# chenhanpolyu/fuxi-planner

Measured on AMD Instinct MI355X. Metric: start->goal plans/sec on 1024x1024 grid, higher is better.
Workload: dtype f64

## Files before the change

### fuxi-planner_amd/_lib.py

```python
import ctypes as C
import os

_HERE = os.path.dirname(os.path.abspath(__file__))
LIB_PATH = os.environ.get("FXJPS_LIB") or os.path.join(_HERE, "libfxjps.so")

OK = 0
E_ARG, E_NODEV, E_HIP, E_NOGRID, E_NOMEM, E_COMM = -1, -2, -3, -4, -5, -6
Q_NOPATH, Q_PATH_TOO_LONG, Q_BAD_START, Q_CAPACITY = 0, -1, -2, -3
BACKEND_HIP = 1

VERSION = 870
PATH_VALID, PATH_EMPTY, PATH_BLOCKED, PATH_OUTSIDE, PATH_MALFORMED = 1, 0, 2, 3, -1
SYMBOLS = ("fxjps_version", "fxjps_timing_size", "fxjps_last_timing_sized", "fxjps_rank_preflight", "fxjps_reserve_grid",
           "fxjps_device_count", "fxjps_create", "fxjps_rank_unique_id", "fxjps_create_rank", "fxjps_set_grid_rank", "fxjps_destroy", "fxjps_last_error",
           "fxjps_set_grid", "fxjps_set_grid_device", "fxjps_prepare_grid", "fxjps_prepare_occupancy_msg", "fxjps_get_grid", "fxjps_get_grid_context", "fxjps_publish_map", "fxjps_set_grid_image", "fxjps_snapshot_image", "fxjps_update_cells", "fxjps_update_cells_deferred", "fxjps_set_queries", "fxjps_replan_frame", "fxjps_plan_batch",
           "fxjps_plan_batch_csr", "fxjps_last_cells", "fxjps_last_timing", "fxjps_last_timing_device", "fxjps_comm_info", "fxjps_set_memory_share", "fxjps_selftest_sqrt", "fxjps_selftest_wavemin", "fxjps_selftest_openlist", "fxjps_debug_read_nbmask", "fxjps_debug_read_maps", "fxjps_debug_counters", "fxjps_debug_qstat",
           "fxjps_waypoint_st", "fxjps_waypoint_ccst", "fxjps_waypoint_ccst_batch", "fxjps_waypoint_st_batch",
           "fxjps_set_grid_slot", "fxjps_get_grid_slot", "fxjps_plan_batch_slots_csr", "fxjps_debug_read_slot_maps", "fxjps_debug_read_sets", "fxjps_debug_live_bytes",
           "fxjps_prepare_slots", "fxjps_slot_job_size", "fxjps_waypoint_slots_batch", "fxjps_publish_slots", "fxjps_slot_publish_size",
           "fxjps_tick_outputs_slots", "fxjps_refresh_slots", "fxjps_debug_read_slot_context", "fxjps_replan_slots",
           "fxjps_set_prior_map", "fxjps_get_prior_map", "fxjps_prepare_slots_world", "fxjps_refresh_slots_world", "fxjps_world_job_size",
           "fxjps_prepare_slots_cropped", "fxjps_refresh_slots_cropped", "fxjps_crop_size",
           "fxjps_refresh_grid", "fxjps_refresh_occupancy_msg", "fxjps_last_refresh_cells", "fxjps_replan_frame_raw",
           "fxjps_set_grid_slots", "fxjps_refresh_grid_slots", "fxjps_grid_job_size",
           "fxjps_set_slot_reuse", "fxjps_debug_slot_tiles", "fxjps_debug_slot_read_sets",
           "fxjps_check_path", "fxjps_check_paths_slots",
# ... 2 lines not shown
           "fxjps_absorb_prior_slide", "fxjps_slide_check", "fxjps_prior_keep_size", "fxjps_prior_slid_size")
MAX_GRID_SLOTS = 256
MAX_PRIOR_MAPS = 16
ABSORB_OVERWRITE, ABSORB_OCCUPIED, ABSORB_KNOWN = 0, 1, 2
ABSORB_MODES = {"overwrite": ABSORB_OVERWRITE, "occupied": ABSORB_OCCUPIED, "known": ABSORB_KNOWN}
KEEP_NONE, KEEP_ALWAYS, KEEP_OVER_LIMIT = 0, 1, 2
KEEP_USES = {"none": KEEP_NONE, "always": KEEP_ALWAYS, "over_limit": KEEP_OVER_LIMIT}
JOB_NOT_PLANNED = 1


class Timing(C.Structure):
    _fields_ = [("search_kernel_ms", C.c_double), ("total_ms", C.c_double), ("search_launches", C.c_int64),
                ("retried", C.c_int64), ("pops", C.c_int64), ("pushes", C.c_int64), ("far_refills", C.c_int64),
                ("slow_pops", C.c_int64), ("table_wipes", C.c_int64), ("reused", C.c_int64), ("table_direct", C.c_int64),
                ("waves", C.c_int64), ("waves_short", C.c_int64), ("head_launch_ms", C.c_double), ("batch_launch_ms", C.c_double),
                ("solo_timeouts", C.c_int64)]


class SlotJob(C.Structure):
    _fields_ = [("raw", C.c_void_p), ("slot", C.c_int32), ("layout", C.c_int32), ("W0", C.c_int32), ("H0", C.c_int32),
                ("ifa", C.c_int32), ("variant", C.c_int32), ("start_xy", C.c_int32 * 2), ("goal_xy", C.c_int32 * 2),
                ("W", C.c_int32), ("H", C.c_int32), ("map_d", C.c_int32 * 2), ("end_occu", C.c_int32), ("status", C.c_int32)]


class GridJob(C.Structure):
    _fields_ = [("occ", C.POINTER(C.c_uint8)), ("slot", C.c_int32), ("W", C.c_int32), ("H", C.c_int32), ("reserved", C.c_int32)]


class WorldJob(C.Structure):
    _fields_ = [("raw", C.c_void_p), ("slot", C.c_int32), ("layout", C.c_int32), ("W0", C.c_int32), ("H0", C.c_int32),
                ("ifa", C.c_int32), ("variant", C.c_int32), ("prior", C.c_int32), ("status", C.c_int32),
# ... 283 lines not shown
```

### fuxi-planner_amd/csrc/fxjps.hip

```cpp
#include <hip/hip_runtime.h>

#include <dlfcn.h>

#include <algorithm>
#include <atomic>
#include <chrono>
#include <cmath>
#include <cstdarg>
#include <cstddef>
#include <cstdio>
#include <cstdlib>
#include <cstring>
#include <mutex>
#include <string>
#include <thread>
#include <vector>

#include "../../include/fxjps.h"
#include "fxjps_kernels.hip.inc"
#include "fxjps_owned.h"
#include "fxjps_results.h"

namespace {

using fx::FarEnt;
using fx::GridDev;
using fx::SearchArgs;
using fx::TEnt;

thread_local std::string g_create_error;

bool dbg_on() {
    static int on = -1;
// ... 87 lines not shown
            **w = 0u;
            g_live_pinned += BYTES;
        } else {
            *w = nullptr;
        }
        return e;
    }
    static void destroy(uint32_t* w) {
        (void)hipHostFree(w);
        g_live_pinned -= BYTES;
    }
};
using Stream = fx::Owned<StreamRes>;
using Event = fx::Owned<EventRes>;
using MappedWord = fx::Owned<MappedWordRes>;

struct ScratchCfg {
    uint32_t nwaves = 0;
    uint32_t nbuckets = 0;
    uint32_t usable = 0;
    uint32_t direct_ly = 0;
    uint32_t far_cap = 0;
};

struct GridBufs {
    int W = 0, H = 0, PW = 0, PH = 0, NS = 0, LINES = 0, WORDS = 0, tsh = 0;
    DBuf<uint8_t> occ, nb8;
    DBuf<fx::BmWord> bm;
    DBuf<int> comp;
    DBuf<uint16_t> ci;
// ... 110 lines not shown
    std::vector<uint32_t> h_order;
    int64_t q0 = 0, nq = 0;
    int wall_khz = 100000;
    struct RunStats {
        double kernel_ms = 0;
        int64_t launches = 0, retried = 0;
        int64_t nrun = 0;
        uint32_t waves_used = 0;
        bool waves_short = false;
        bool had_solo = false;
        double head_ms = 0, batch_ms = 0;
    } run;
    HBuf<uint8_t> h_absorb_in;
    DBuf<uint8_t> d_absorb_in;
    HBuf<unsigned long long> h_absorb_out;

    DevCtx() = default;
    DevCtx(DevCtx&&) = default;
    DevCtx& operator=(DevCtx&&) = default;
    ~DevCtx() {
        if (dev < 0) return;
        (void)hipSetDevice(dev);
        if (stream_solo) (void)hipStreamSynchronize(stream_solo);
        if (stream) (void)hipStreamSynchronize(stream);
    }
};

}

struct fxjps {
    std::vector<DevCtx> devs;
    std::string err;
    std::mutex err_mu;
    bool have_grid = false;
    bool maps_stale = false;
    int mem_div = 1;
    fxjps_timing_t timing{};
// ... 60 lines not shown
        h->err = buf;
    } else {
        g_create_error = buf;
    }
    return code;
}

#define HIPCHK(h, call)                                                                          \
    do {                                                                                         \
        hipError_t e__ = (call);                                                                 \
        if (e__ != hipSuccess)                                                                   \
            return fail(h, e__ == hipErrorOutOfMemory ? FXJPS_E_NOMEM : FXJPS_E_HIP, "%s: %s (%s:%d)", \
                        #call, hipGetErrorString(e__), __FILE__, __LINE__);                      \
    } while (0)

uint32_t dirlut_entry(uint32_t pd, uint32_t nbm) {
    auto occ = [&](int dx, int dy) -> bool { return (nbm >> fx::nbit(dx, dy)) & 1u; };
    auto blocked = [&](int dx, int dy) -> bool {
        if (dx != 0 && dy != 0) return (occ(dx, 0) && occ(0, dy)) || occ(dx, dy);
        return occ(dx, dy);
    };
    uint32_t codes[8];
    int n = 0;
    auto add = [&](int dx, int dy) { codes[n++] = (uint32_t)((dx + 1) * 4 + (dy + 1)); };
    const int pdx = (int)(pd >> 2) - 1, pdy = (int)(pd & 3u) - 1;
    if (pd == fx::PD_NONE) {
        static const int all8[8][2] = {{-1, 0}, {0, -1}, {1, 0}, {0, 1}, {-1, -1}, {-1, 1}, {1, -1}, {1, 1}};
        for (auto& d : all8)
            if (!blocked(d[0], d[1])) add(d[0], d[1]);
    } else if (pdx < -1 || pdx > 1 || pdy < -1 || pdy > 1) {
    } else if (pdx != 0 && pdy != 0) {
        if (!blocked(0, pdy)) add(0, pdy);
        if (!blocked(pdx, 0)) add(pdx, 0);
        if ((!blocked(0, pdy) || !blocked(pdx, 0)) && !blocked(pdx, pdy)) add(pdx, pdy);
        if (blocked(-pdx, 0) && !blocked(0, pdy)) add(-pdx, pdy);
        if (blocked(0, -pdy) && !blocked(pdx, 0)) add(pdx, -pdy);
    } else if (pdx == 0) {
        if (!blocked(0, pdy)) add(0, pdy);
        if (blocked(1, 0)) add(1, pdy);
        if (blocked(-1, 0)) add(-1, pdy);
    } else {
        if (!blocked(pdx, 0)) {
            add(pdx, 0);
            if (blocked(0, 1)) add(pdx, 1);
            if (blocked(0, -1)) add(pdx, -1);
        }
    }
    uint32_t v = 0;
    for (int g = 0; g < 8; g++) v |= (g < n ? codes[g] : fx::DIR_NONE) << (4 * g);
    return v;
}

GridDev grid_of(const GridBufs& d) {
    GridDev G;
    G.bm = d.bm.p;
    G.ci = d.ci.p;
    G.nb8 = d.nb8.p;
    G.jd = d.jd.p;
    G.comp = d.comp.p;
    G.W = d.W;
    G.H = d.H;
    G.PW = d.PW;
    G.PH = d.PH;
    G.NS = d.NS;
    G.LINES = d.LINES;
    G.WORDS = d.WORDS;
    G.DLINES = d.PW + d.PH - 1;
    G.tsh = d.tsh;
    return G;
}

int derive_maps(fxjps* h, DevCtx& d, bool whole = true, GridBufs* slot = nullptr) {
    HIPCHK(h, hipSetDevice(d.dev));
    GridBufs& g = slot ? *slot : d;
    if (slot) whole = true;
    if (!whole && !d.dirty && !d.ccl_full) return FXJPS_OK;
    const bool box = !whole && d.dirty && (d.bx1 - d.bx0 + 1) * 2 <= g.PW && (d.by1 - d.by0 + 1) * 2 <= g.PH;
    const GridDev G = grid_of(g);
    const char* fused_env = getenv("FXJPS_FUSED_BUILD");
    if (whole && !(fused_env && atoi(fused_env) == 0) && (long long)g.W * g.H <= (1ll << 18)) {
        const long long ncell = (long long)g.W * g.H, npad = (long long)g.PW * g.PH;
        const unsigned nb_rows = (unsigned)(((long long)g.PW * g.WORDS + 3) / 4), nb_cols = (unsigned)(((long long)g.PH * g.WORDS + 3) / 4);
        const unsigned nb_cell = (unsigned)((ncell + 255) / 256), nb_ci = (unsigned)((npad + 255) / 256);
        const unsigned nb_diag = (unsigned)((4ll * G.DLINES * g.WORDS + 15) / 16), nb_flat = (unsigned)((ncell + 1023) / 1024);
        hipLaunchKernelGGL(fx::k_build_1, dim3(nb_rows + nb_cols + nb_cell), dim3(256), 0, d.stream, g.occ.p, G, g.nb8.p, g.bm.p, g.comp.p, nb_rows, nb_cols);
        hipLaunchKernelGGL(fx::k_build_2, dim3(nb_ci + nb_cell), dim3(256), 0, d.stream, g.occ.p, G, g.ci.p, g.comp.p, nb_ci);
        hipLaunchKernelGGL(fx::k_build_3, dim3(nb_diag + nb_flat), dim3(1024), 0, d.stream, g.occ.p, G, g.bm.p + (size_t)4 * g.LINES * g.WORDS, g.comp.p, nb_diag);
        hipLaunchKernelGGL(fx::k_derive_jd, dim3((unsigned)((npad * 8 + 255) / 256)), dim3(256), 0, d.stream, G, g.jd.p, fx::DiagRange{1, d.bx0, d.bx1, d.by0, d.by1});
        HIPCHK(h, hipGetLastError());
        if (!slot) {
// ... 107 lines not shown
    d.LINES = std::max(d.PW, d.PH);
    d.WORDS = (std::max(d.PW, d.PH) + 63) / 64;
    d.tsh = 0;
    while (((std::max(W, H) - 1) >> d.tsh) > 63) d.tsh++;
    HIPCHK(h, d.occ.ensure((size_t)W * H));
    HIPCHK(h, d.comp.ensure((size_t)W * H));
    HIPCHK(h, d.nb8.ensure((size_t)d.PW * d.NS));
    HIPCHK(h, d.ci.ensure((size_t)d.PW * d.NS));
    HIPCHK(h, d.jd.ensure((size_t)d.PW * d.NS * 8));
    HIPCHK(h, d.bm.ensure((size_t)4 * d.LINES * d.WORDS + (size_t)4 * (d.PW + d.PH - 1) * d.WORDS));
    return FXJPS_OK;
}

int alloc_grid(fxjps* h, DevCtx& d, int W, int H) {
    HIPCHK(h, hipSetDevice(d.dev));
    bool knob = false;
    for (const char* k : {"FXJPS_TABLE_LOG2", "FXJPS_TABLE_SHIFT", "FXJPS_FAR_CAP", "FXJPS_POOL_BUDGET_MB", "FXJPS_POOL_FRAC", "FXJPS_DIRECT",
                          "FXJPS_TABLE_SHRINK"})
        knob = knob || getenv(k) != nullptr;
    if (W != d.W || H != d.H || knob) {
        d.pool_clean[0] = d.pool_clean[1] = false;
        d.cfg[0] = ScratchCfg();
        d.cfg[1] = ScratchCfg();
        d.owner_ready = false;
        d.chg_ready = false;
    }
    return alloc_grid_bufs(h, d, W, H);
}

constexpr uint64_t wpb_down(uint64_t v) { return v / (uint64_t)fx::WPB * (uint64_t)fx::WPB; }
// ... 202 lines not shown
    A.max_pops = 64ull * (unsigned long long)req.cells + 4096ull;
    if (req.slots) {
        A.grids = d.d_slot_desc.p;
        A.grid_ids = d.d_grid_ids.p;
    }
    if (d.st.on) {
        A.host_cells = d.st.cells;
        A.host_cap = d.st.cap;
        A.host_cursor = d.d_cursor.p;
        A.host_base = d.st.base;
        A.host_len = d.st.len;
        A.host_cost = d.st.cost;
    }
}

int launch_search(fxjps* h, DevCtx& d, const BatchReq& req, int pool, const uint32_t* d_order, uint32_t nrun) {
    const ScratchCfg& c = d.cfg[pool];
    const bool track = req.track();
    SearchArgs A;
    fill_search_args(d, req, pool, A, d_order, nrun);
    uint32_t waves = std::min<uint32_t>(c.nwaves, (nrun + 0u));
    waves = std::max<uint32_t>((uint32_t)fx::WPB, (uint32_t)wpb_up(waves));
    waves = std::min<uint32_t>(waves, c.nwaves);
    uint32_t nsolo = (nrun <= 32768u && d.share * h->mem_div == 1) ? 16u : 0u, live_solo = 1, live_main = 0;
    if (const char* e = getenv("FXJPS_SOLO")) nsolo = (uint32_t)std::max(0, atoi(e));
    if (const char* e = getenv("FXJPS_SOLO_LIVE")) live_solo = (uint32_t)std::max(1, atoi(e));
    if (const char* e = getenv("FXJPS_SPREAD")) live_main = (uint32_t)std::max(0, atoi(e));
    if (live_solo != 1u && live_solo != 2u && live_solo != 4u) live_solo = 4u;
    if (live_main != 0u && live_main != 1u && live_main != 2u && live_main != 4u) live_main = 4u;
    if (pool != 0 || track || d_order == nullptr || d.solo_started == nullptr || d.solo_timeouts_run >= 3 || nrun < 4096u || nrun < 64u * nsolo ||
        waves <= 2u * nsolo + (uint32_t)fx::WPB)
        nsolo = 0;
    nsolo = std::min<uint32_t>(nsolo, 512u) & ~(live_solo - 1u);
    if (nsolo != 0u) waves = std::min<uint32_t>(waves, (uint32_t)wpb_down(c.nwaves - nsolo));

    if (pool != 0 || nsolo != 0u || (uint64_t)nrun > (uint64_t)d.n_cu * live_main || d.share * h->mem_div > 1) live_main = 0u;
    if (pool == 0) d.run.waves_used = waves;
    HIPCHK(h, hipMemsetAsync(d.d_next.p, 0, 4 * sizeof(unsigned int), d.stream));
    const dim3 block(fx::WAVE * fx::WPB);
    DBG("launch k_search pool=%d waves=%u nrun=%u buckets=%u far_cap=%u solo=%u x %u spread=%u", pool, waves, nrun, c.nbuckets, c.far_cap, nsolo,
        live_solo, live_main);
    HIPCHK(h, hipEventRecord(d.ev0, d.stream));
    {
        const SearchKernel k = search_kernel(req.hchoice, track, c.direct_ly > 0, req.slots);
        const SearchFn fn = k.fn;
        static const size_t pad = 36u << 10;
        if (nsolo != 0u || live_main != 0u) {
            if (!d.lds_attr_done[k.index]) {
                if (hipFuncSetAttribute(reinterpret_cast<const void*>(fn), hipFuncAttributeMaxDynamicSharedMemorySize, (int)pad) == hipSuccess) {
// ... 41 lines not shown
            hipLaunchKernelGGL(fn, dim3(waves / fx::WPB), block, 0, d.stream, A);
        }
        HIPCHK(h, hipGetLastError());
        if (nsolo != 0u) {
            HIPCHK(h, hipEventRecord(d.ev_bt1, d.stream));
            HIPCHK(h, hipStreamWaitEvent(d.stream, d.ev_solo1, 0));
        }
        if (pool == 0) d.run.had_solo = nsolo != 0u;
    }
    HIPCHK(h, hipEventRecord(d.ev1, d.stream));
    if (d.st.on) {
        hipLaunchKernelGGL(fx::k_counters_out, dim3(1), dim3(64), 0, d.stream, d.d_counters.p, d.st.counters);
        HIPCHK(h, hipGetLastError());
    }
    d.run.launches += nsolo != 0u ? 2 : 1;
    return FXJPS_OK;
}

constexpr size_t ARENA_BYTES = (size_t)1 << 30;
int begin_streaming(fxjps* h, DevCtx& d, const BatchReq& req) {
    const int64_t nq = d.nq;
    const unsigned long long limit = ARENA_BYTES / sizeof(uint32_t) / h->devs.size();
    unsigned long long want = (unsigned long long)nq * (unsigned long long)std::min(req.max_len, 512);
    want = std::max(want, (unsigned long long)d.arena_peak + (unsigned long long)d.arena_peak / 4);
    if (const char* e = getenv("FXJPS_ARENA_CELLS")) want = (unsigned long long)std::max(0ll, atoll(e));
    if (want > limit) return FXJPS_OK;
    HIPCHK(h, d.h_arena.ensure((size_t)std::max(want, 1ull)));
    HIPCHK(h, d.h_base.ensure((size_t)nq));
    HIPCHK(h, d.d_cursor.ensure(1));
    void *dp_cells = nullptr, *dp_base = nullptr, *dp_len = nullptr, *dp_cost = nullptr, *dp_cnt = nullptr;
// ... 82 lines not shown
    int rc = ensure_pool(h, d, req, 0, (uint32_t)std::min<int64_t>(full, (d.run.nrun + 3) & ~3ll));
    if (rc) return rc;
    DBG("pool ready");
    if (req.stream && d.cfg[0].direct_ly > 0)
        if ((rc = begin_streaming(h, d, req)) != FXJPS_OK) return rc;
    return launch_search(h, d, req, 0, d.d_order.p, (uint32_t)d.run.nrun);
}

int finish_search(fxjps* h, DevCtx& d, const BatchReq& req) {
    HIPCHK(h, hipSetDevice(d.dev));
    const int64_t nq = d.nq;
    if (nq == 0) return FXJPS_OK;
    DBG("waiting for the search kernel");
    HIPCHK(h, hipStreamSynchronize(d.stream));
    DBG("search kernel done");
    if (!d.st.on) {
        HIPCHK(h, hipMemcpyAsync(d.h_len.p, d.d_len.p, (size_t)nq * sizeof(int32_t), hipMemcpyDeviceToHost, d.stream));
        HIPCHK(h, hipStreamSynchronize(d.stream));
    }
    float ms = 0;
    if (d.run.launches > 0) {
        HIPCHK(h, hipEventElapsedTime(&ms, d.ev0, d.ev1));
        d.run.kernel_ms += ms;
        if (d.run.had_solo) {
            float a = 0, b = 0;
            HIPCHK(h, hipEventElapsedTime(&a, d.ev_hd0, d.ev_hd1));
            HIPCHK(h, hipEventElapsedTime(&b, d.ev_bt0, d.ev_bt1));
            d.run.head_ms = a;
            d.run.batch_ms = b;
        }
// ... 308 lines not shown
    T.search_kernel_ms = 0;
    T.search_launches = 0;
    T.retried = 0;
    T.pops = 0;
    T.pushes = 0;
    T.far_refills = 0;
    T.slow_pops = 0;
    T.table_wipes = 0;
    T.reused = 0;
    T.table_direct = 0;
    T.waves = 0;
    T.waves_short = 0;
    T.head_launch_ms = 0;
    T.batch_launch_ms = 0;
    T.solo_timeouts = 0;
    for (auto& d : h->devs) {
        T.head_launch_ms = std::max(T.head_launch_ms, d.run.head_ms);
        T.batch_launch_ms = std::max(T.batch_launch_ms, d.run.batch_ms);
        T.solo_timeouts += d.solo_timeouts;
        T.waves += d.run.waves_used;
        if (d.run.waves_short) T.waves_short = 1;
        T.search_kernel_ms = std::max(T.search_kernel_ms, d.run.kernel_ms);
        T.search_launches += d.run.launches;
        T.retried += d.run.retried;
        if (d.nq > 0) {
            T.pops += (int64_t)d.h_counters.p[0];
            T.pushes += (int64_t)d.h_counters.p[1];
            T.far_refills += (int64_t)d.h_counters.p[2];
            T.slow_pops += (int64_t)d.h_counters.p[3];
            T.table_wipes += (int64_t)d.h_counters.p[7];
            if (d.cfg[0].direct_ly > 0) T.table_direct = 1;
// ... 90 lines not shown
        if (rc) return rc;
    }
    for (auto& d : h->devs) {
        if (!wait) break;
        HIPCHK(h, hipSetDevice(d.dev));
        HIPCHK(h, hipStreamSynchronize(d.stream));
    }
    h->have_grid = true;
    h->maps_stale = false;
    return FXJPS_OK;
}

void drain_all(fxjps* h) {
    const std::string keep = h->err;
    for (auto& d : h->devs) {
        if (hipSetDevice(d.dev) == hipSuccess) {
            if (d.stream_solo) (void)hipStreamSynchronize(d.stream_solo);
            (void)hipStreamSynchronize(d.stream);
        }
        d.pool_clean[0] = d.pool_clean[1] = false;
        d.owner_ready = d.chg_ready = false;
    }
    (void)hipGetLastError();
    h->err = keep;
}

struct WpPaths {
    struct Part {
        DevCtx* d;
        int64_t q0, n, total, kept_at;
        const long long* h_off;
// ... 677 lines not shown
    HIPCHK(h, hipSetDevice(d.dev));
    const size_t n = (size_t)d.W * d.H * channels;
    HIPCHK(h, d.d_img.ensure(n));
    int rc = transpose_map(h, d, d.occ.p, d.W, d.H, 0, 1, fx::TM_OCC_TO_GRAY, channels, d.d_img.p);
    if (rc) return rc;
    HIPCHK(h, hipMemcpyAsync(out, d.d_img.p, n, hipMemcpyDeviceToHost, d.stream));
    HIPCHK(h, hipStreamSynchronize(d.stream));
    return FXJPS_OK;
}

namespace {
int update_cells_async(fxjps_t* h, const int32_t* xy, const uint8_t* val, int64_t n, bool derive) {
    if (!h->have_grid) return fail(h, FXJPS_E_NOGRID, "cell update before fxjps_set_grid");
    if (n < 0 || n > 0x7FFFFFF0ll || (n > 0 && (!xy || !val))) return fail(h, FXJPS_E_ARG, "bad update arrays");
    if (n == 0 && !(derive && h->maps_stale)) return FXJPS_OK;
    int bx0 = 0, bx1 = -1, by0 = 0, by1 = -1;
    bool have_box = false;
    {
        const DevCtx& d0 = h->devs[0];
        for (int64_t i = 0; i < n; i++) {
            const int x = xy[2 * i], y = xy[2 * i + 1];
            if (x < 0 || y < 0 || x >= d0.W || y >= d0.H) continue;
            bx0 = have_box ? std::min(bx0, x) : x;
            bx1 = have_box ? std::max(bx1, x) : x;
            by0 = have_box ? std::min(by0, y) : y;
            by1 = have_box ? std::max(by1, y) : y;
            have_box = true;
        }
    }
    static const bool partial = !(getenv("FXJPS_PARTIAL_DERIVE") && atoi(getenv("FXJPS_PARTIAL_DERIVE")) == 0);
// ... 2757 lines not shown
```

### fuxi-planner_amd/csrc/fxjps_kernels.hip.inc

```

namespace fx {

constexpr int WAVE = 64;
#define FX_RARE(c) __builtin_expect(!!(c), 0)
#define FX_USUAL(c) __builtin_expect(!!(c), 1)
#ifndef FXJPS_WPB
#define FXJPS_WPB 8
#endif
#ifndef FXJPS_OCC
#define FXJPS_OCC 4
#endif
constexpr int WPB = FXJPS_WPB;
constexpr int OCC = FXJPS_OCC;
constexpr uint32_t KEY_CLOSED = 0x80000000u;
constexpr uint32_t CELL_MASK = 0x03FFFFFFu;
constexpr uint32_t PD_NONE = 5;
constexpr uint32_t SLOT_NONE = 0xFFFFFFFFu;
constexpr uint32_t PAR_MASK = 0x07FFFFFFu;
constexpr uint32_t PAR_NONE = PAR_MASK;
constexpr uint32_t GEN_WRAP = 63u;
__host__ __device__ constexpr uint32_t ent_gen(uint32_t key, uint32_t par) { return ((key >> 30) & 1u) | ((par >> 27) << 1); }
__host__ __device__ constexpr uint32_t gen_key_bits(uint32_t gen) { return (gen & 1u) << 30; }
__host__ __device__ constexpr uint32_t gen_par_bits(uint32_t gen) { return (gen >> 1) << 27; }
constexpr uint32_t DIR_NONE = 0xFu;
// ... 2875 lines not shown
    }
    if (lane == 0) {
        out_info[0] = total;
        out_info[1] = fail;
        out_info[4] = (uint32_t)Q.r_n;
        out_info[5] = Q.m_n;
        out_info[6] = Q.far_n;
        out_info[7] = Q.farb_n;
    }
}

__global__ __launch_bounds__(64) void k_counters_out(const unsigned long long* __restrict__ counters, unsigned long long* __restrict__ host) {
    host[threadIdx.x] = counters[threadIdx.x];
}

__global__ __launch_bounds__(1024) void k_scan_len(const int32_t* __restrict__ len, long long nq,
                                                   long long* __restrict__ offsets) {
    __shared__ long long s_part[1024];
    const int tid = threadIdx.x;
    const long long per = (nq + 1023) / 1024;
    const long long lo = (long long)tid * per, hi = min(lo + per, nq);
    long long sum = 0;
    for (long long i = lo; i < hi; i++) sum += len[i] > 0 ? len[i] : 0;
    s_part[tid] = sum;
    __syncthreads();
    for (int o = 1; o < 1024; o <<= 1) {
        long long v = tid >= o ? s_part[tid - o] : 0;
        __syncthreads();
        s_part[tid] += v;
        __syncthreads();
// ... 126 lines not shown
```

### include/fxjps.h

```cpp
#ifndef FXJPS_H
#define FXJPS_H

#include <stdint.h>

#ifdef __cplusplus
extern "C" {
#endif

#if defined(__GNUC__) || defined(__clang__)
#pragma GCC visibility push(default)
#endif

typedef struct fxjps fxjps_t;

#define FXJPS_OK 0
#define FXJPS_E_ARG (-1)
#define FXJPS_E_NODEV (-2)
#define FXJPS_E_HIP (-3)
#define FXJPS_E_NOGRID (-4)
#define FXJPS_E_NOMEM (-5)
#define FXJPS_E_COMM (-6)

#define FXJPS_Q_NOPATH 0
#define FXJPS_Q_PATH_TOO_LONG (-1)
#define FXJPS_Q_BAD_START (-2)
#define FXJPS_Q_CAPACITY (-3)

#define FXJPS_BACKEND_HIP 1

#define FXJPS_VERSION 870
int fxjps_version(void);

int fxjps_device_count(void);

int fxjps_create(int backend, const int* device_ids, int n_dev, fxjps_t** out);

int fxjps_rank_unique_id(void* out_id128);
int fxjps_create_rank(int device, int rank, int world, const void* id128, fxjps_t** out);
int fxjps_set_grid_rank(fxjps_t* h, const uint8_t* occ, int32_t W, int32_t H);
int fxjps_rank_preflight(int device);
int fxjps_reserve_grid(fxjps_t* h, int32_t W, int32_t H);

void fxjps_destroy(fxjps_t* h);

const char* fxjps_last_error(fxjps_t* h);
// ... 226 lines not shown
    double total_ms;
    int64_t search_launches;
    int64_t retried;
    int64_t pops;
    int64_t pushes;
    int64_t far_refills;
    int64_t slow_pops;
    int64_t table_wipes;
    int64_t reused;
    int64_t table_direct;
    int64_t waves;
    int64_t waves_short;
    double head_launch_ms;
    double batch_launch_ms;
    int64_t solo_timeouts;
} fxjps_timing_t;
int fxjps_last_timing(fxjps_t* h, fxjps_timing_t* out);
int fxjps_timing_size(void);
int fxjps_last_timing_sized(fxjps_t* h, void* out, int64_t out_size);

int fxjps_last_timing_device(fxjps_t* h, int32_t ctx, int32_t* out_device, int64_t* out_nq, double* out_kernel_ms,
                             int64_t* out_waves);

int fxjps_comm_info(fxjps_t* h, int32_t* out_contexts, int32_t* out_devices, int32_t* out_rccl_ranks);

int fxjps_set_memory_share(fxjps_t* h, int32_t handles_per_device);

int fxjps_selftest_sqrt(fxjps_t* h, uint32_t n0, uint32_t n1, double* out);

int fxjps_selftest_wavemin(fxjps_t* h, int32_t rounds, uint64_t seed, int64_t* mismatches);
// ... 66 lines not shown
```

Before: 155,400.

## Offload tail of hardest queries to host CPU threads during GPU search

Adds a host-side JPS searcher and runs the first few queries of the work order (by default 16, on 8 threads) on CPU threads in parallel with the GPU search kernel. The maps are copied to pinned host memory once per map generation, and the CPU results are scattered into the device output buffers by a small kernel. The point is to remove the long-tail queries that keep the GPU busy with a few slow waves. In exchange it adds thread synchronisation, host copies whenever the map changes, and an adaptive cap that shrinks the host share when the host finishes late.

```diff
diff --git a/fuxi-planner_amd/_lib.py b/fuxi-planner_amd/_lib.py
--- a/fuxi-planner_amd/_lib.py
+++ b/fuxi-planner_amd/_lib.py
@@ -9,7 +9,7 @@
 Q_NOPATH, Q_PATH_TOO_LONG, Q_BAD_START, Q_CAPACITY = 0, -1, -2, -3
 BACKEND_HIP = 1
 
-VERSION = 870
+VERSION = 880
 PATH_VALID, PATH_EMPTY, PATH_BLOCKED, PATH_OUTSIDE, PATH_MALFORMED = 1, 0, 2, 3, -1
 SYMBOLS = ("fxjps_version", "fxjps_timing_size", "fxjps_last_timing_sized", "fxjps_rank_preflight", "fxjps_reserve_grid",
            "fxjps_device_count", "fxjps_create", "fxjps_rank_unique_id", "fxjps_create_rank", "fxjps_set_grid_rank", "fxjps_destroy", "fxjps_last_error",
@@ -42,7 +42,8 @@
                 ("retried", C.c_int64), ("pops", C.c_int64), ("pushes", C.c_int64), ("far_refills", C.c_int64),
                 ("slow_pops", C.c_int64), ("table_wipes", C.c_int64), ("reused", C.c_int64), ("table_direct", C.c_int64),
                 ("waves", C.c_int64), ("waves_short", C.c_int64), ("head_launch_ms", C.c_double), ("batch_launch_ms", C.c_double),
-                ("solo_timeouts", C.c_int64)]
+                ("solo_timeouts", C.c_int64), ("host_tail_queries", C.c_int64), ("host_tail_ms", C.c_double),
+                ("host_tail_late", C.c_int64)]
 
 
 class SlotJob(C.Structure):
diff --git a/fuxi-planner_amd/csrc/fxjps.hip b/fuxi-planner_amd/csrc/fxjps.hip
--- a/fuxi-planner_amd/csrc/fxjps.hip
+++ b/fuxi-planner_amd/csrc/fxjps.hip
@@ -6,17 +6,20 @@
 #include <atomic>
 #include <chrono>
 #include <cmath>
+#include <condition_variable>
 #include <cstdarg>
 #include <cstddef>
 #include <cstdio>
 #include <cstdlib>
 #include <cstring>
+#include <memory>
 #include <mutex>
 #include <string>
 #include <thread>
 #include <vector>
 
 #include "../../include/fxjps.h"
+#include "fxjps_host_search.h"
 #include "fxjps_kernels.hip.inc"
 #include "fxjps_owned.h"
 #include "fxjps_results.h"
@@ -134,6 +137,110 @@
 using Stream = fx::Owned<StreamRes>;
 using Event = fx::Owned<EventRes>;
 using MappedWord = fx::Owned<MappedWordRes>;
+
+constexpr uint32_t HOST_TAIL_MAX = 64, HOST_TAIL_THREADS_MAX = 12;
+struct HostTail {
+    uint32_t kh_cap = HOST_TAIL_MAX;
+    int late_run = 0;
+    int ontime_run = 0;
+    uint64_t maps_gen = ~0ull;
+    fxh::Maps maps;
+    HBuf<uint16_t> jd;
+    HBuf<fx::BmWord> bm;
+    HBuf<int32_t> comp;
+    Stream stream;
+    Event ev_grid, ev_maps;
+    std::vector<uint32_t> lut;
+    std::vector<std::unique_ptr<fxh::Searcher>> searchers;
+    HBuf<uint32_t> path, ids;
+    HBuf<int32_t> len;
+    HBuf<double> cost;
+    std::vector<std::thread> threads;
+    std::mutex mu;
+    std::condition_variable cv;
+    int go = 0;
+    std::atomic<uint32_t> next{0}, ended{0};
+    std::atomic<bool> cancel{false};
+    std::atomic<unsigned long long> pops{0}, pushes{0};
+    double t_first = 0, t_last = 0;
+    uint32_t kh = 0;
+    const int32_t *starts = nullptr, *goals = nullptr;
+    const uint32_t* order = nullptr;
+    int hchoice = 0, max_len = 0;
+    uint64_t max_pops = 0;
+    uint32_t done_kh = 0;
+    double done_ms = 0;
+    bool done_late = false;
+
+    void work(size_t t) {
+        {
+            std::unique_lock<std::mutex> lk(mu);
+            cv.wait(lk, [&] { return go != 0; });
+            if (go < 0) return;
+        }
+        const double t0 = now_s();
+        try {
+            for (uint32_t i = next.fetch_add(1); i < kh && !cancel.load(std::memory_order_relaxed); i = next.fetch_add(1)) {
+                const uint32_t q = order[i];
+                const fxh::Result R = searchers[t]->plan(maps, lut.data(), hchoice, starts[2 * q], starts[2 * q + 1], goals[2 * q], goals[2 * q + 1],
+                                                         max_len, path.p + (size_t)i * (size_t)max_len, max_pops);
+                cost.p[i] = R.cost;
+                len.p[i] = R.len;
+                pops += R.pops;
+                pushes += R.pushes;
+            }
+        } catch (...) {
+        }
+        const double t1 = now_s();
+        std::lock_guard<std::mutex> lk(mu);
+        t_first = ended.load() == 0 ? t0 : std::min(t_first, t0);
+        t_last = ended.load() == 0 ? t1 : std::max(t_last, t1);
+        ended++;
+    }
+    bool spawn(size_t T) {
+        go = 0;
+        next = 0;
+        ended = 0;
+        cancel = false;
+        pops = 0;
+        pushes = 0;
+        try {
+            if (lut.empty()) {
+                lut.resize(11 * 256);
+                fxh::dirlut_fill(lut.data());
+            }
+            while (searchers.size() < T) searchers.emplace_back(new fxh::Searcher());
+            threads.reserve(T);
+            for (size_t t = 0; t < T; t++) threads.emplace_back([this, t] { work(t); });
+        } catch (...) {
+            release(-1);
+            return false;
+        }
+        return true;
+    }
+    void release(int how) {
+        {
+            std::lock_guard<std::mutex> lk(mu);
+            go = how;
+        }
+        cv.notify_all();
+        if (how < 0) join();
+    }
+    void join() {
+        for (auto& t : threads)
+            if (t.joinable()) t.join();
+        threads.clear();
+    }
+    void abandon() {
+        if (threads.empty()) return;
+        cancel = true;
+        release(go == 0 ? -1 : go);
+        join();
+        kh = 0;
+        maps_gen = ~0ull;
+    }
+    ~HostTail() { abandon(); }
+};
 
 struct ScratchCfg {
     uint32_t nwaves = 0;
@@ -274,13 +381,17 @@
     HBuf<uint8_t> h_absorb_in;
     DBuf<uint8_t> d_absorb_in;
     HBuf<unsigned long long> h_absorb_out;
+    uint64_t map_gen = 0;
+    std::unique_ptr<HostTail> tail;
 
     DevCtx() = default;
     DevCtx(DevCtx&&) = default;
     DevCtx& operator=(DevCtx&&) = default;
     ~DevCtx() {
+        if (tail) tail->abandon();
         if (dev < 0) return;
         (void)hipSetDevice(dev);
+        if (tail && tail->stream) (void)hipStreamSynchronize(tail->stream);
         if (stream_solo) (void)hipStreamSynchronize(stream_solo);
         if (stream) (void)hipStreamSynchronize(stream);
     }
@@ -371,42 +482,10 @@
                         #call, hipGetErrorString(e__), __FILE__, __LINE__);                      \
     } while (0)
 
-uint32_t dirlut_entry(uint32_t pd, uint32_t nbm) {
-    auto occ = [&](int dx, int dy) -> bool { return (nbm >> fx::nbit(dx, dy)) & 1u; };
-    auto blocked = [&](int dx, int dy) -> bool {
-        if (dx != 0 && dy != 0) return (occ(dx, 0) && occ(0, dy)) || occ(dx, dy);
-        return occ(dx, dy);
-    };
-    uint32_t codes[8];
-    int n = 0;
-    auto add = [&](int dx, int dy) { codes[n++] = (uint32_t)((dx + 1) * 4 + (dy + 1)); };
-    const int pdx = (int)(pd >> 2) - 1, pdy = (int)(pd & 3u) - 1;
-    if (pd == fx::PD_NONE) {
-        static const int all8[8][2] = {{-1, 0}, {0, -1}, {1, 0}, {0, 1}, {-1, -1}, {-1, 1}, {1, -1}, {1, 1}};
-        for (auto& d : all8)
-            if (!blocked(d[0], d[1])) add(d[0], d[1]);
-    } else if (pdx < -1 || pdx > 1 || pdy < -1 || pdy > 1) {
-    } else if (pdx != 0 && pdy != 0) {
-        if (!blocked(0, pdy)) add(0, pdy);
-        if (!blocked(pdx, 0)) add(pdx, 0);
-        if ((!blocked(0, pdy) || !blocked(pdx, 0)) && !blocked(pdx, pdy)) add(pdx, pdy);
-        if (blocked(-pdx, 0) && !blocked(0, pdy)) add(-pdx, pdy);
-        if (blocked(0, -pdy) && !blocked(pdx, 0)) add(pdx, -pdy);
-    } else if (pdx == 0) {
-        if (!blocked(0, pdy)) add(0, pdy);
-        if (blocked(1, 0)) add(1, pdy);
-        if (blocked(-1, 0)) add(-1, pdy);
-    } else {
-        if (!blocked(pdx, 0)) {
-            add(pdx, 0);
-            if (blocked(0, 1)) add(pdx, 1);
-            if (blocked(0, -1)) add(pdx, -1);
-        }
-    }
-    uint32_t v = 0;
-    for (int g = 0; g < 8; g++) v |= (g < n ? codes[g] : fx::DIR_NONE) << (4 * g);
-    return v;
-}
+using fxh::dirlut_entry;
+static_assert(fxh::PD_NONE == fx::PD_NONE && fxh::DIR_NONE == fx::DIR_NONE && fxh::QI_WATCHDOG == fx::QI_WATCHDOG &&
+                  sizeof(fxh::BmWord) == sizeof(fx::BmWord),
+              "the host search reads the device's maps and codes");
 
 GridDev grid_of(const GridBufs& d) {
     GridDev G;
@@ -431,6 +510,7 @@
     HIPCHK(h, hipSetDevice(d.dev));
     GridBufs& g = slot ? *slot : d;
     if (slot) whole = true;
+    if (!slot) d.map_gen++;
     if (!whole && !d.dirty && !d.ccl_full) return FXJPS_OK;
     const bool box = !whole && d.dirty && (d.bx1 - d.bx0 + 1) * 2 <= g.PW && (d.by1 - d.by0 + 1) * 2 <= g.PH;
     const GridDev G = grid_of(g);
@@ -568,6 +648,7 @@
 
 int alloc_grid(fxjps* h, DevCtx& d, int W, int H) {
     HIPCHK(h, hipSetDevice(d.dev));
+    d.map_gen++;
     bool knob = false;
     for (const char* k : {"FXJPS_TABLE_LOG2", "FXJPS_TABLE_SHIFT", "FXJPS_FAR_CAP", "FXJPS_POOL_BUDGET_MB", "FXJPS_POOL_FRAC", "FXJPS_DIRECT",
                           "FXJPS_TABLE_SHRINK"})
@@ -800,6 +881,119 @@
     }
 }
 
+constexpr uint32_t HOST_TAIL_DEFAULT = 16, HOST_TAIL_THREADS_DEFAULT = 8;
+uint32_t host_tail_begin(fxjps* h, DevCtx& d, const BatchReq& req, const ScratchCfg& c) {
+    uint32_t kh = HOST_TAIL_DEFAULT, T = HOST_TAIL_THREADS_DEFAULT;
+    if (d.tail) d.tail->done_kh = 0;
+    const char* named = getenv("FXJPS_HOST_TAIL");
+    if (named) kh = (uint32_t)std::min(std::max(0, atoi(named)), (int)HOST_TAIL_MAX);
+    if (const char* e = getenv("FXJPS_HOST_THREADS")) T = (uint32_t)std::min(std::max(1, atoi(e)), (int)HOST_TAIL_THREADS_MAX);
+    if (kh == 0u || h->devs.size() != 1 || c.direct_ly == 0u || req.slots || req.track() || d.st.on || getenv("FXJPS_QSTAT") ||
+        req.max_len > (1 << 16) || req.cells > (1ull << 20))
+        return 0u;
+    if (!d.tail) {
+        try {
+            d.tail.reset(new HostTail());
+        } catch (...) {
+            return 0u;
+        }
+    }
+    HostTail& t = *d.tail;
+    t.abandon();
+    if (!named) {
+        kh = std::min(kh, t.kh_cap);
+        if (t.late_run >= 3 || kh == 0u) return 0u;
+    }
+    T = std::min(T, kh);
+    const bool copy = t.maps_gen != d.map_gen;
+    bool ok = t.path.ensure((size_t)kh * (size_t)req.max_len) == hipSuccess && t.ids.ensure(kh) == hipSuccess && t.len.ensure(kh) == hipSuccess &&
+              t.cost.ensure(kh) == hipSuccess;
+    if (ok && copy) {
+        t.maps_gen = ~0ull;
+        ok = t.jd.ensure((size_t)d.PW * d.NS * 8) == hipSuccess && t.bm.ensure((size_t)4 * d.LINES * d.WORDS) == hipSuccess &&
+             t.comp.ensure((size_t)d.W * d.H) == hipSuccess && (t.stream || t.stream.create(hipStreamNonBlocking) == hipSuccess) &&
+             (t.ev_grid || t.ev_grid.create(hipEventDisableTiming) == hipSuccess) && (t.ev_maps || t.ev_maps.create(hipEventDisableTiming) == hipSuccess) &&
+             hipEventRecord(t.ev_grid, d.stream) == hipSuccess;
+    }
+    if (!ok) {
+        (void)hipGetLastError();
+        return 0u;
+    }
+    for (uint32_t i = 0; i < kh; i++) {
+        t.ids.p[i] = d.h_order[i];
+        t.len.p[i] = fx::QI_WATCHDOG;
+        t.cost.p[i] = 0.0;
+    }
+    t.starts = req.starts + 2 * d.q0;
+    t.goals = req.goals + 2 * d.q0;
+    t.order = d.h_order.data();
+    t.hchoice = req.hchoice;
+    t.max_len = req.max_len;
+    t.max_pops = 64ull * (unsigned long long)req.cells + 4096ull;
+    t.kh = kh;
+    if (!t.spawn(T)) {
+        t.kh = 0;
+        return 0u;
+    }
+    return kh;
+}
+
+int host_tail_go(fxjps* h, DevCtx& d) {
+    HostTail& t = *d.tail;
+    if (t.maps_gen != d.map_gen) {
+        HIPCHK(h, hipStreamWaitEvent(t.stream, t.ev_grid, 0));
+        HIPCHK(h, hipMemcpyAsync(t.jd.p, d.jd.p, (size_t)d.PW * d.NS * 8 * sizeof(uint16_t), hipMemcpyDeviceToHost, t.stream));
+        HIPCHK(h, hipMemcpyAsync(t.bm.p, d.bm.p, (size_t)4 * d.LINES * d.WORDS * sizeof(fx::BmWord), hipMemcpyDeviceToHost, t.stream));
+        HIPCHK(h, hipMemcpyAsync(t.comp.p, d.comp.p, (size_t)d.W * d.H * sizeof(int32_t), hipMemcpyDeviceToHost, t.stream));
+        HIPCHK(h, hipEventRecord(t.ev_maps, t.stream));
+        HIPCHK(h, hipEventSynchronize(t.ev_maps));
+        t.maps.jd = t.jd.p;
+        t.maps.bm = reinterpret_cast<const fxh::BmWord*>(t.bm.p);
+        t.maps.comp = t.comp.p;
+        t.maps.W = d.W;
+        t.maps.H = d.H;
+        t.maps.NS = d.NS;
+        t.maps.LINES = d.LINES;
+        t.maps.WORDS = d.WORDS;
+        t.maps_gen = d.map_gen;
+    }
+    t.release(1);
+    return FXJPS_OK;
+}
+
+int host_tail_end(fxjps* h, DevCtx& d, const BatchReq& req) {
+    HostTail& t = *d.tail;
+    const uint32_t kh = t.kh;
+    const bool late = t.ended.load() < (uint32_t)t.threads.size();
+    t.join();
+    t.kh = 0;
+    if (late) {
+        t.kh_cap = std::max(1u, std::min(t.kh_cap, kh) / 2u);
+        t.late_run++;
+        t.ontime_run = 0;
+    } else {
+        t.late_run = 0;
+        if (++t.ontime_run >= 16) {
+            t.kh_cap = std::min(HOST_TAIL_MAX, t.kh_cap * 2u);
+            t.ontime_run = 0;
+        }
+    }
+    t.done_kh = kh;
+    t.done_ms = (t.t_last - t.t_first) * 1e3;
+    t.done_late = late;
+    void *dp_ids = nullptr, *dp_path = nullptr, *dp_len = nullptr, *dp_cost = nullptr;
+    HIPCHK(h, hipHostGetDevicePointer(&dp_ids, t.ids.p, 0));
+    HIPCHK(h, hipHostGetDevicePointer(&dp_path, t.path.p, 0));
+    HIPCHK(h, hipHostGetDevicePointer(&dp_len, t.len.p, 0));
+    HIPCHK(h, hipHostGetDevicePointer(&dp_cost, t.cost.p, 0));
+    hipLaunchKernelGGL(fx::k_host_tail_put, dim3(kh), dim3(256), 0, d.stream, (const uint32_t*)dp_ids, (const uint32_t*)dp_path, (const int32_t*)dp_len,
+                       (const double*)dp_cost, req.max_len, (long long)d.nq, d.d_path.p, d.d_len.p, d.d_cost.p, d.d_counters.p,
+                       (unsigned long long)t.pops.load(), (unsigned long long)t.pushes.load());
+    HIPCHK(h, hipGetLastError());
+    DBG("host tail: %u queries, %.3f ms%s", kh, t.done_ms, late ? " (late)" : "");
+    return FXJPS_OK;
+}
+
 int launch_search(fxjps* h, DevCtx& d, const BatchReq& req, int pool, const uint32_t* d_order, uint32_t nrun) {
     const ScratchCfg& c = d.cfg[pool];
     const bool track = req.track();
@@ -819,6 +1013,13 @@
         nsolo = 0;
     nsolo = std::min<uint32_t>(nsolo, 512u) & ~(live_solo - 1u);
     if (nsolo != 0u) waves = std::min<uint32_t>(waves, (uint32_t)wpb_down(c.nwaves - nsolo));
+    const uint32_t kh = nsolo != 0u ? host_tail_begin(h, d, req, c) : 0u;
+    if (kh != 0u) {
+        d_order += kh;
+        nrun -= kh;
+        A.order = d_order;
+        A.nrun = nrun;
+    }
 
     if (pool != 0 || nsolo != 0u || (uint64_t)nrun > (uint64_t)d.n_cu * live_main || d.share * h->mem_div > 1) live_main = 0u;
     if (pool == 0) d.run.waves_used = waves;
@@ -890,6 +1091,7 @@
         HIPCHK(h, hipGetLastError());
     }
     d.run.launches += nsolo != 0u ? 2 : 1;
+    if (kh != 0u) return host_tail_go(h, d);
     return FXJPS_OK;
 }
 
@@ -1002,6 +1204,8 @@
     DBG("waiting for the search kernel");
     HIPCHK(h, hipStreamSynchronize(d.stream));
     DBG("search kernel done");
+    if (d.tail && d.tail->kh != 0u)
+        if (int rc = host_tail_end(h, d, req)) return rc;
     if (!d.st.on) {
         HIPCHK(h, hipMemcpyAsync(d.h_len.p, d.d_len.p, (size_t)nq * sizeof(int32_t), hipMemcpyDeviceToHost, d.stream));
         HIPCHK(h, hipStreamSynchronize(d.stream));
@@ -1340,7 +1544,15 @@
     T.head_launch_ms = 0;
     T.batch_launch_ms = 0;
     T.solo_timeouts = 0;
+    T.host_tail_queries = 0;
+    T.host_tail_ms = 0;
+    T.host_tail_late = 0;
     for (auto& d : h->devs) {
+        if (d.tail && d.tail->done_kh != 0u && d.nq > 0 && d.run.had_solo) {
+            T.host_tail_queries += d.tail->done_kh;
+            T.host_tail_ms = std::max(T.host_tail_ms, d.tail->done_ms);
+            if (d.tail->done_late) T.host_tail_late = 1;
+        }
         T.head_launch_ms = std::max(T.head_launch_ms, d.run.head_ms);
         T.batch_launch_ms = std::max(T.batch_launch_ms, d.run.batch_ms);
         T.solo_timeouts += d.solo_timeouts;
@@ -1461,7 +1673,9 @@
 void drain_all(fxjps* h) {
     const std::string keep = h->err;
     for (auto& d : h->devs) {
+        if (d.tail) d.tail->abandon();
         if (hipSetDevice(d.dev) == hipSuccess) {
+            if (d.tail && d.tail->stream) (void)hipStreamSynchronize(d.tail->stream);
             if (d.stream_solo) (void)hipStreamSynchronize(d.stream_solo);
             (void)hipStreamSynchronize(d.stream);
         }
@@ -2169,6 +2383,7 @@
     if (!h->have_grid) return fail(h, FXJPS_E_NOGRID, "cell update before fxjps_set_grid");
     if (n < 0 || n > 0x7FFFFFF0ll || (n > 0 && (!xy || !val))) return fail(h, FXJPS_E_ARG, "bad update arrays");
     if (n == 0 && !(derive && h->maps_stale)) return FXJPS_OK;
+    for (auto& d : h->devs) d.map_gen++;
     int bx0 = 0, bx1 = -1, by0 = 0, by1 = -1;
     bool have_box = false;
     {
diff --git a/fuxi-planner_amd/csrc/fxjps_host_search.cpp b/fuxi-planner_amd/csrc/fxjps_host_search.cpp
--- /dev/null
+++ b/fuxi-planner_amd/csrc/fxjps_host_search.cpp
@@ -0,0 +1,297 @@
+#include "fxjps_host_search.h"
+
+#include <cmath>
+#include <cstdlib>
+#include <cstring>
+
+namespace fxh {
+
+namespace {
+
+constexpr uint32_t JD_K = 0x1FFFu, JD_J = 0x8000u;
+constexpr uint32_t NO_PARENT = 0xFFFFFFFFu;
+
+constexpr int nbit(int dx, int dy) { return ((dx + 1) * 3 + (dy + 1)) - ((((dx + 1) * 3 + (dy + 1)) > 4) ? 1 : 0); }
+constexpr uint32_t jd_slot(uint32_t code) { return code - (code >= 3u ? 1u : 0u) - (code >= 5u ? 1u : 0u) - (code >= 7u ? 1u : 0u); }
+
+inline uint64_t bits_of(double v) {
+    uint64_t b;
+    std::memcpy(&b, &v, sizeof b);
+    return b;
+}
+
+template <int HC>
+inline double heuristic(int ax, int ay, int bx, int by) {
+    if (HC == 1) {
+        const int xd = std::abs(bx - ax), yd = std::abs(by - ay);
+        return (double)(xd > yd ? 14 * yd + 10 * (xd - yd) : 14 * xd + 10 * (yd - xd));
+    }
+    const int dx = bx - ax, dy = by - ay;
+    return std::sqrt((double)(uint32_t)(dx * dx + dy * dy));
+}
+template <int HC>
+inline double seg_len(int cx, int cy, int jx, int jy) {
+    const int lx = std::abs(cx - jx), ly = std::abs(cy - jy);
+    if (HC == 1) return (lx != 0 && ly != 0) ? (double)(lx * 14) : (double)((lx + ly) * 10);
+    return std::sqrt((double)(uint32_t)(lx * lx + ly * ly));
+}
+
+inline bool scan_line(const Maps& M, int di, int line, int pos, int gpos) {
+    const int sgn = (di & 1) ? -1 : 1;
+    const BmWord* L = M.bm + (size_t)(di * M.LINES + line) * M.WORDS;
+    int w = pos >> 6;
+    const int b = pos & 63;
+    uint64_t m = sgn > 0 ? (~0ull << b) : (~0ull >> (63 - b));
+    const int gw = gpos >> 6;
+    const uint64_t gbit = gpos >= 0 ? (1ull << (gpos & 63)) : 0ull;
+    while (w >= 0 && w < M.WORDS) {
+        const BmWord u = L[w];
+        uint64_t s = u.stop;
+        if (w == gw) s |= gbit;
+        s &= m;
+        if (s) {
+            const int bit = sgn > 0 ? __builtin_ctzll(s) : 63 - __builtin_clzll(s);
+            return !((u.occ >> bit) & 1ull);
+        }
+        w += sgn;
+        m = ~0ull;
+    }
+    return false;
+}
+inline bool scan_ray(const Maps& M, int px, int py, int dx, int dy, int gpx, int gpy) {
+    if (dx != 0) return scan_line(M, dx > 0 ? 0 : 1, py, px + dx, py == gpy ? gpx : -1);
+    return scan_line(M, dy > 0 ? 2 : 3, px, py + dy, px == gpx ? gpy : -1);
+}
+inline bool scan_two(const Maps& M, int ox, int oy, int dx, int dy, int gpx, int gpy) {
+    return scan_ray(M, ox, oy, dx, 0, gpx, gpy) || scan_ray(M, ox, oy, 0, dy, gpx, gpy);
+}
+
+inline bool expand_ray(const Maps& M, const uint16_t* rec, int cpx, int cpy, uint32_t code, int gpx, int gpy, int* jxp, int* jyp) {
+    const int dx = (int)(code >> 2) - 1, dy = (int)(code & 3u) - 1;
+    const bool diag = dx != 0 && dy != 0, alongY = dx == 0;
+    const uint32_t v = rec[jd_slot(code) & 7u];
+    const int ax = dx > 0 ? gpx - cpx : cpx - gpx, ay = dy > 0 ? gpy - cpy : cpy - gpy;
+    const bool gline = diag ? (ax == ay) : (alongY ? gpx == cpx : gpy == cpy);
+    const int kg = alongY ? ay : ax;
+    const int k = (int)(v & JD_K);
+    const bool jp = (v & JD_J) != 0u;
+    const bool goal_on = gline && kg >= 1 && kg <= k;
+    bool has = goal_on ? (kg < k ? true : jp) : jp;
+    int kres = goal_on ? kg : k;
+    if (diag && ((ax >= 1 && ax < kres) || (ay >= 1 && ay < kres))) {
+        const int k1 = ax < ay ? ax : ay, k2 = ax < ay ? ay : ax;
+        if (k1 >= 1 && k1 < kres && scan_two(M, cpx + k1 * dx, cpy + k1 * dy, dx, dy, gpx, gpy)) {
+            has = true;
+            kres = k1;
+        } else if (k2 != k1 && k2 >= 1 && k2 < kres && scan_two(M, cpx + k2 * dx, cpy + k2 * dy, dx, dy, gpx, gpy)) {
+            has = true;
+            kres = k2;
+        }
+    }
+    *jxp = cpx + kres * dx;
+    *jyp = cpy + kres * dy;
+    return has;
+}
+
+inline bool occupied(const Maps& M, int x, int y) {
+    return (M.bm[(size_t)(2 * M.LINES + x + 1) * M.WORDS + ((y + 1) >> 6)].occ >> ((y + 1) & 63)) & 1ull;
+}
+
+}
+
+uint32_t dirlut_entry(uint32_t pd, uint32_t nbm) {
+    auto occ = [&](int dx, int dy) -> bool { return (nbm >> nbit(dx, dy)) & 1u; };
+    auto blocked = [&](int dx, int dy) -> bool {
+        if (dx != 0 && dy != 0) return (occ(dx, 0) && occ(0, dy)) || occ(dx, dy);
+        return occ(dx, dy);
+    };
+    uint32_t codes[8];
+    int n = 0;
+    auto add = [&](int dx, int dy) { codes[n++] = (uint32_t)((dx + 1) * 4 + (dy + 1)); };
+    const int pdx = (int)(pd >> 2) - 1, pdy = (int)(pd & 3u) - 1;
+    if (pd == PD_NONE) {
+        static const int all8[8][2] = {{-1, 0}, {0, -1}, {1, 0}, {0, 1}, {-1, -1}, {-1, 1}, {1, -1}, {1, 1}};
+        for (auto& d : all8)
+            if (!blocked(d[0], d[1])) add(d[0], d[1]);
+    } else if (pdx < -1 || pdx > 1 || pdy < -1 || pdy > 1) {
+    } else if (pdx != 0 && pdy != 0) {
+        if (!blocked(0, pdy)) add(0, pdy);
+        if (!blocked(pdx, 0)) add(pdx, 0);
+        if ((!blocked(0, pdy) || !blocked(pdx, 0)) && !blocked(pdx, pdy)) add(pdx, pdy);
+        if (blocked(-pdx, 0) && !blocked(0, pdy)) add(-pdx, pdy);
+        if (blocked(0, -pdy) && !blocked(pdx, 0)) add(pdx, -pdy);
+    } else if (pdx == 0) {
+        if (!blocked(0, pdy)) add(0, pdy);
+        if (blocked(1, 0)) add(1, pdy);
+        if (blocked(-1, 0)) add(-1, pdy);
+    } else {
+        if (!blocked(pdx, 0)) {
+            add(pdx, 0);
+            if (blocked(0, 1)) add(pdx, 1);
+            if (blocked(0, -1)) add(pdx, -1);
+        }
+    }
+    uint32_t v = 0;
+    for (int g = 0; g < 8; g++) v |= (g < n ? codes[g] : DIR_NONE) << (4 * g);
+    return v;
+}
+
+void dirlut_fill(uint32_t* lut) {
+    for (uint32_t pd = 0; pd < 11; pd++)
+        for (uint32_t m = 0; m < 256; m++) lut[pd * 256 + m] = dirlut_entry(pd, m);
+}
+
+static inline bool key_less(uint64_t af, uint32_t ac, uint64_t bf, uint32_t bc) { return af < bf || (af == bf && ac < bc); }
+
+void Searcher::heap_push(HeapEnt e) {
+    size_t i = heap_.size();
+    heap_.push_back(e);
+    HeapEnt* a = heap_.data();
+    while (i > 0) {
+        const size_t p = (i - 1) >> 1;
+        if (!key_less(e.f, e.cell, a[p].f, a[p].cell)) break;
+        a[i] = a[p];
+        i = p;
+    }
+    a[i] = e;
+}
+
+Searcher::HeapEnt Searcher::heap_pop() {
+    HeapEnt* a = heap_.data();
+    const HeapEnt top = a[0];
+    const HeapEnt last = heap_.back();
+    heap_.pop_back();
+    const size_t n = heap_.size();
+    if (n > 0) {
+        size_t i = 0;
+        for (;;) {
+            size_t c = 2 * i + 1;
+            if (c >= n) break;
+            if (c + 1 < n && key_less(a[c + 1].f, a[c + 1].cell, a[c].f, a[c].cell)) c++;
+            if (!key_less(a[c].f, a[c].cell, last.f, last.cell)) break;
+            a[i] = a[c];
+            i = c;
+        }
+        a[i] = last;
+    }
+    return top;
+}
+
+template <int HC>
+Result Searcher::search(const Maps& M, const uint32_t* dirlut, int sx, int sy, int gx, int gy, int max_len, uint32_t* out_path, uint64_t max_pops) {
+    Result R;
+    const int H = M.H;
+    const size_t ncell = (size_t)M.W * (size_t)H;
+    if (tab_.size() != ncell || gen_ >= 0x7FFFFFFEu) {
+        tab_.assign(ncell, Ent{0.0, NO_PARENT, 0u});
+        gen_ = 0;
+    }
+    gen_++;
+    const uint32_t live = gen_ << 1;
+    Ent* tab = tab_.data();
+    heap_.clear();
+    const int gpx = gx + 1, gpy = gy + 1;
+    const uint32_t sidx = (uint32_t)(sx * H + sy), goal_cell = ((uint32_t)gx << 13) | (uint32_t)gy;
+    tab[sidx] = Ent{0.0, NO_PARENT, live};
+    heap_push(HeapEnt{bits_of(heuristic<HC>(sx, sy, gx, gy)), ((uint32_t)sx << 13) | (uint32_t)sy, sidx});
+    while (!heap_.empty()) {
+        const HeapEnt cur = heap_pop();
+        R.pops++;
+        if (R.pops > max_pops) {
+            R.len = QI_WATCHDOG;
+            return R;
+        }
+        const Ent ec = tab[cur.idx];
+        if (cur.cell == goal_cell) {
+            R.cost = ec.g;
+            walk_.clear();
+            uint32_t i = cur.idx;
+            for (;;) {
+                walk_.push_back(i);
+                if (i == sidx) break;
+                i = tab[i].par;
+            }
+            const size_t n = walk_.size();
+            if (n > (size_t)max_len) {
+                R.len = Q_PATH_TOO_LONG;
+                return R;
+            }
+            for (size_t k = 0; k < n; k++) {
+                const uint32_t c = walk_[n - 1 - k];
+                out_path[k] = ((c / (uint32_t)H) << 16) | (c % (uint32_t)H);
+            }
+            R.len = (int32_t)n;
+            return R;
+        }
+        if (ec.tag & 1u) continue;
+        tab[cur.idx].tag = live | 1u;
+        const int cx = (int)(cur.cell >> 13), cy = (int)(cur.cell & 0x1FFFu);
+        uint32_t pd = PD_NONE;
+        if (ec.par != NO_PARENT) {
+            const int px = (int)(ec.par / (uint32_t)H), py = (int)(ec.par % (uint32_t)H);
+            const int ddx = cx > px ? 1 : (cx < px ? -1 : 0), ddy = cy > py ? 1 : (cy < py ? -1 : 0);
+            pd = (uint32_t)((ddx + 1) * 4 + (ddy + 1));
+        }
+        const uint16_t* rec = M.jd + ((size_t)(cx + 1) * (size_t)M.NS + (size_t)(cy + 1)) * 8u;
+        const uint32_t nb8 = ((rec[0] >> 13) & 3u) | (((rec[1] >> 13) & 3u) << 2) | (((rec[2] >> 13) & 3u) << 4) | (((rec[3] >> 13) & 3u) << 6);
+        uint32_t codes = dirlut[pd * 256u + nb8];
+        for (int ray = 0; ray < 8; ray++, codes >>= 4) {
+            const uint32_t code = codes & 0xFu;
+            if (code == DIR_NONE) break;
+            int jxp, jyp;
+            if (!expand_ray(M, rec, cx + 1, cy + 1, code, gpx, gpy, &jxp, &jyp)) continue;
+            const int jx = jxp - 1, jy = jyp - 1;
+            const uint32_t jidx = (uint32_t)(jx * H + jy);
+            Ent& ej = tab[jidx];
+            const bool seen = (ej.tag >> 1) == gen_;
+            if (seen && (ej.tag & 1u)) continue;
+            const double tg = ec.g + seg_len<HC>(cx, cy, jx, jy);
+            if (!seen || tg < ej.g) {
+                ej = Ent{tg, cur.idx, live};
+                const double f = tg + heuristic<HC>(jx, jy, gx, gy);
+                heap_push(HeapEnt{bits_of(f), ((uint32_t)jx << 13) | (uint32_t)jy, jidx});
+                R.pushes++;
+            }
+        }
+    }
+    return R;
+}
+
+Result Searcher::plan(const Maps& M, const uint32_t* dirlut, int hchoice, int sx, int sy, int gx, int gy, int max_len, uint32_t* out_path,
+                      uint64_t max_pops) {
+    Result R;
+    if (sx < 0 || sy < 0 || sx >= M.W || sy >= M.H) {
+        R.len = Q_BAD_START;
+        return R;
+    }
+    if (sx == gx && sy == gy) {
+        if (max_len < 1) {
+            R.len = Q_PATH_TOO_LONG;
+            return R;
+        }
+        out_path[0] = ((uint32_t)sx << 16) | (uint32_t)sy;
+        R.len = 1;
+        return R;
+    }
+    if (gx < 0 || gy < 0 || gx >= M.W || gy >= M.H) return R;
+    if (occupied(M, gx, gy)) return R;
+    if (M.comp != nullptr && !occupied(M, sx, sy)) {
+        const auto root = [&](int i) -> int {
+            int p = M.comp[i];
+            if (p < 0) return -1;
+            for (int step = 0; step < 256 && p != i; step++) {
+                i = p;
+                p = M.comp[i];
+            }
+            return p == i ? i : -2;
+        };
+        const int cs = root(sx * M.H + sy), cg = root(gx * M.H + gy);
+        if (cs >= 0 && cg >= 0 && cg != cs) return R;
+    }
+    R = hchoice == 1 ? search<1>(M, dirlut, sx, sy, gx, gy, max_len, out_path, max_pops)
+                     : search<2>(M, dirlut, sx, sy, gx, gy, max_len, out_path, max_pops);
+    if (R.len == 0 || R.len <= QI_WATCHDOG) R.cost = 0.0;
+    return R;
+}
+
+}
diff --git a/fuxi-planner_amd/csrc/fxjps_host_search.h b/fuxi-planner_amd/csrc/fxjps_host_search.h
--- /dev/null
+++ b/fuxi-planner_amd/csrc/fxjps_host_search.h
@@ -0,0 +1,57 @@
+#pragma once
+#include <cstdint>
+#include <vector>
+
+namespace fxh {
+
+struct BmWord {
+    uint64_t stop, occ;
+};
+
+struct Maps {
+    const uint16_t* jd = nullptr;
+    const BmWord* bm = nullptr;
+    const int32_t* comp = nullptr;
+    int32_t W = 0, H = 0, NS = 0, LINES = 0, WORDS = 0;
+};
+
+constexpr uint32_t PD_NONE = 5, DIR_NONE = 0xFu;
+constexpr int32_t Q_PATH_TOO_LONG = -1, Q_BAD_START = -2, QI_WATCHDOG = -102;
+
+uint32_t dirlut_entry(uint32_t pd, uint32_t nbm);
+void dirlut_fill(uint32_t* lut);
+
+struct Result {
+    int32_t len = 0;
+    double cost = 0.0;
+    uint64_t pops = 0, pushes = 0;
+};
+
+class Searcher {
+public:
+    Result plan(const Maps& M, const uint32_t* dirlut, int hchoice, int sx, int sy, int gx, int gy, int max_len, uint32_t* out_path,
+                uint64_t max_pops);
+
+private:
+    struct Ent {
+        double g;
+        uint32_t par;
+        uint32_t tag;
+    };
+    struct HeapEnt {
+        uint64_t f;
+        uint32_t cell;
+        uint32_t idx;
+    };
+    template <int HC>
+    Result search(const Maps& M, const uint32_t* dirlut, int sx, int sy, int gx, int gy, int max_len, uint32_t* out_path, uint64_t max_pops);
+    void heap_push(HeapEnt e);
+    HeapEnt heap_pop();
+
+    std::vector<Ent> tab_;
+    std::vector<HeapEnt> heap_;
+    std::vector<uint32_t> walk_;
+    uint32_t gen_ = 0;
+};
+
+}
diff --git a/fuxi-planner_amd/csrc/fxjps_kernels.hip.inc b/fuxi-planner_amd/csrc/fxjps_kernels.hip.inc
--- a/fuxi-planner_amd/csrc/fxjps_kernels.hip.inc
+++ b/fuxi-planner_amd/csrc/fxjps_kernels.hip.inc
@@ -2913,6 +2913,25 @@
     host[threadIdx.x] = counters[threadIdx.x];
 }
 
+__global__ __launch_bounds__(256) void k_host_tail_put(const uint32_t* __restrict__ ids, const uint32_t* __restrict__ path, const int32_t* __restrict__ len,
+                                                       const double* __restrict__ cost, int max_len, long long nq, uint32_t* __restrict__ out_path,
+                                                       int32_t* __restrict__ out_len, double* __restrict__ out_cost,
+                                                       unsigned long long* __restrict__ counters, unsigned long long pops, unsigned long long pushes) {
+    const uint32_t i = blockIdx.x, q = ids[i];
+    if (i == 0u && threadIdx.x == 0u) {
+        counters[0] += pops;
+        counters[1] += pushes;
+    }
+    if ((long long)q >= nq) return;
+    const int32_t n = len[i];
+    const int cells = n < 0 ? 0 : (n > max_len ? max_len : n);
+    for (int k = (int)threadIdx.x; k < cells; k += 256) out_path[(size_t)q * (size_t)max_len + (size_t)k] = path[(size_t)i * (size_t)max_len + (size_t)k];
+    if (threadIdx.x == 0u) {
+        out_len[q] = n;
+        out_cost[q] = cost[i];
+    }
+}
+
 __global__ __launch_bounds__(1024) void k_scan_len(const int32_t* __restrict__ len, long long nq,
                                                    long long* __restrict__ offsets) {
     __shared__ long long s_part[1024];
diff --git a/include/fxjps.h b/include/fxjps.h
--- a/include/fxjps.h
+++ b/include/fxjps.h
@@ -28,7 +28,7 @@
 
 #define FXJPS_BACKEND_HIP 1
 
-#define FXJPS_VERSION 870
+#define FXJPS_VERSION 880
 int fxjps_version(void);
 
 int fxjps_device_count(void);
@@ -285,6 +285,9 @@
     double head_launch_ms;
     double batch_launch_ms;
     int64_t solo_timeouts;
+    int64_t host_tail_queries;
+    double host_tail_ms;
+    int64_t host_tail_late;
 } fxjps_timing_t;
 int fxjps_last_timing(fxjps_t* h, fxjps_timing_t* out);
 int fxjps_timing_size(void);
```

After: 168,300, median of 6. 1.08x the previous value.
